# Azure/mmlspark

Measured on NVIDIA H100. Metric: boosting_iters_per_sec, higher is better.
Workload: dtype int64 fixed-point histograms over u8 bins (fp32 gradients, fp64 split gains)

## Files before the change

include/b200gbm_c_api.h:

```cpp
#ifndef B200GBM_C_API_H_
#define B200GBM_C_API_H_

#include <stddef.h>
#include <stdint.h>

#ifdef __cplusplus
extern "C" {
#endif

typedef void* DatasetHandle;
typedef void* BoosterHandle;

#define C_API_DTYPE_FLOAT32 (0)
#define C_API_DTYPE_FLOAT64 (1)
#define C_API_DTYPE_INT32 (2)
#define C_API_DTYPE_INT64 (3)

#define C_API_PREDICT_NORMAL (0)
#define C_API_PREDICT_RAW_SCORE (1)
#define C_API_PREDICT_LEAF_INDEX (2)
#define C_API_PREDICT_CONTRIB (3)

const char* LGBM_GetLastError(void);

// ... 51 lines not shown
                          int64_t buffer_len, int64_t* out_len, char* out_str);

int LGBM_BoosterPredictForMatSingle(BoosterHandle handle, const void* data, int data_type, int ncol, int is_row_major,
                                    int predict_type, int start_iteration, int num_iteration, const char* parameter,
                                    int64_t* out_len, double* out_result);
int LGBM_BoosterPredictForCSRSingle(BoosterHandle handle, const void* indptr, int indptr_type, const int32_t* indices,
                                    const void* data, int data_type, int64_t nindptr, int64_t nelem, int64_t num_col,
                                    int predict_type, int start_iteration, int num_iteration, const char* parameter,
                                    int64_t* out_len, double* out_result);
int LGBM_BoosterPredictForMat(BoosterHandle handle, const void* data, int data_type, int32_t nrow, int32_t ncol,
                              int is_row_major, int predict_type, int start_iteration, int num_iteration,
                              const char* parameter, int64_t* out_len, double* out_result);
int LGBM_BoosterCalcNumPredict(BoosterHandle handle, int num_row, int predict_type, int start_iteration,
                               int num_iteration, int64_t* out_len);

typedef void* ChunkedArrayHandle;
int B200GBM_ChunkedArrayCreate(int data_type, int64_t chunk_size, ChunkedArrayHandle* out);
int B200GBM_ChunkedArrayAdd(ChunkedArrayHandle h, double value);
int B200GBM_ChunkedArrayAddMany(ChunkedArrayHandle h, const void* values, int64_t n);
int64_t B200GBM_ChunkedArrayGetAddCount(ChunkedArrayHandle h);
int64_t B200GBM_ChunkedArrayGetChunksCount(ChunkedArrayHandle h);
int64_t B200GBM_ChunkedArrayGetLastChunkAddCount(ChunkedArrayHandle h);
double B200GBM_ChunkedArrayGetItem(ChunkedArrayHandle h, int64_t chunk, int64_t index, double on_fail);
int B200GBM_ChunkedArrayCoalesceTo(ChunkedArrayHandle h, void* out);
int B200GBM_ChunkedArrayRelease(ChunkedArrayHandle h);
int B200GBM_ChunkedArrayFree(ChunkedArrayHandle h);

int B200GBM_SetDevice(int ordinal);
int B200GBM_GetDevice(int* ordinal);
int B200GBM_DeviceAlloc(size_t bytes, void** out);
int B200GBM_DeviceFree(void* ptr);
int B200GBM_HostAllocPinned(size_t bytes, void** out);
int B200GBM_HostFreePinned(void* ptr);
int B200GBM_Memcpy(void* dst, const void* src, size_t bytes);
int B200GBM_SampleIndices(int num_total_row, int sample_cnt, int seed, int* out, int* out_len);
int B200GBM_SyntheticFill(void* dev_x_f32, void* dev_label_f32, int64_t row_start, int32_t nrow, int32_t ncol,
                          uint64_t seed, int kind);
int B200GBM_SyntheticRows(const int* rows, int32_t nrows, int32_t ncol, uint64_t seed, int kind, double* host_out,
                          float* host_label_out);
int B200GBM_DatasetGetBins(DatasetHandle handle, uint8_t* out_row_major);
int B200GBM_DatasetGetBins16(DatasetHandle handle, uint16_t* out_row_major);
int B200GBM_DatasetGetBinToCat(DatasetHandle handle, int feature, int* out, int* out_len);
int B200GBM_DatasetGetBinsRows(DatasetHandle handle, const int32_t* rows, int32_t nrows, uint16_t* out);
int B200GBM_DatasetGetBundles(DatasetHandle handle, int* out_num_columns, int* out_column_of);
int B200GBM_DatasetGetFeatureRange(DatasetHandle handle, int feature, double* out2);
int B200GBM_DatasetGetFeatureInfo(DatasetHandle handle, int feature, int* out5);
int B200GBM_DatasetGetUpperBounds(DatasetHandle handle, int feature, double* out, int* out_len);
int B200GBM_DatasetGetIngestMs(DatasetHandle handle, double* out_ms);
int B200GBM_DatasetHistogram(DatasetHandle handle, const float* grad, const float* hess, const int32_t* idx,
                             int32_t cnt, double* out);
int B200GBM_BoosterGetGradients(BoosterHandle handle, float* grad, float* hess);
int B200GBM_BoosterSetProfile(BoosterHandle handle, int profile_hist);
int B200GBM_BoosterGetTiming(BoosterHandle handle, double* out6, int reset);
int B200GBM_BoosterGetScores(BoosterHandle handle, int data_idx, double* out);
int B200GBM_BoosterPredictForMatDevice(BoosterHandle handle, const void* data, int data_type, int64_t nrow, int32_t ncol, int predict_type,
                                       int start_iteration, int num_iteration, int64_t* out_len, double* out_result, double* elapsed_ms);
int B200GBM_BoosterPredictForCSRDevice(BoosterHandle handle, const void* indptr, int indptr_type, const int32_t* indices, const void* data,
                                       int data_type, int64_t nindptr, int64_t nelem, int64_t num_col, int predict_type, int start_iteration,
                                       int num_iteration, int64_t* out_len, double* out_result, double* elapsed_ms);
int B200GBM_BoosterGetInfo(BoosterHandle handle, int* out4);
int B200GBM_BoosterGetMemoryInfo(BoosterHandle handle, int64_t* out2);
int B200GBM_BoosterGetColumnCacheInfo(BoosterHandle handle, int64_t* out4);
int B200GBM_BoosterGetCommInfo(BoosterHandle handle, int64_t* out3);

#ifdef __cplusplus
}
#endif
#endif
```

mmlspark_b200/capi.py:

```python
import ctypes as C
import os

import numpy as np

_HERE = os.path.dirname(os.path.abspath(__file__))
LIB_PATH = os.path.join(_HERE, "lib", "libb200gbm.so")
_LIB = None

DTYPE_FLOAT32, DTYPE_FLOAT64, DTYPE_INT32, DTYPE_INT64 = 0, 1, 2, 3
PREDICT_NORMAL, PREDICT_RAW_SCORE, PREDICT_LEAF_INDEX, PREDICT_CONTRIB = 0, 1, 2, 3


class LightGBMError(Exception):
    pass


def load():
    global _LIB
    if _LIB is None:
        if not os.path.exists(LIB_PATH):
            raise LightGBMError(
                "libb200gbm.so is missing (%s). Run `python __graft_entry__.py` to build the CUDA extension; "
                "this package has no CPU fallback." % LIB_PATH)
        L = C.CDLL(LIB_PATH, mode=C.RTLD_GLOBAL)
# ... 393 lines not shown
        X = np.ascontiguousarray(X, dtype=np.float64)
        nrow, ncol = X.shape
        n = C.c_int64(0)
        check(load().LGBM_BoosterCalcNumPredict(self.handle, C.c_int(nrow), C.c_int(predict_type), C.c_int(start_iteration), C.c_int(num_iteration), C.byref(n)))
        out = np.zeros(max(n.value, 1), dtype=np.float64)
        check(load().LGBM_BoosterPredictForMat(self.handle, _ptr(X), C.c_int(DTYPE_FLOAT64), C.c_int32(nrow), C.c_int32(ncol), C.c_int(1), C.c_int(predict_type),
                                               C.c_int(start_iteration), C.c_int(num_iteration), b"", C.byref(n), _ptr(out)))
        return out[:n.value].reshape(nrow, -1)

    def predict_device(self, X, predict_type=PREDICT_NORMAL, start_iteration=0, num_iteration=-1, return_ms=False):
        X = np.ascontiguousarray(X)
        if X.dtype not in (np.float32, np.float64):
            X = X.astype(np.float64)
        nrow, ncol = X.shape
        n = C.c_int64(0)
        check(load().LGBM_BoosterCalcNumPredict(self.handle, C.c_int(nrow), C.c_int(predict_type), C.c_int(start_iteration), C.c_int(num_iteration), C.byref(n)))
        out = np.zeros(max(n.value, 1), dtype=np.float64)
        ms = C.c_double(0)
        check(load().B200GBM_BoosterPredictForMatDevice(self.handle, _ptr(X), C.c_int(_np_dtype_code(X)), C.c_int64(nrow), C.c_int32(ncol), C.c_int(predict_type),
                                                        C.c_int(start_iteration), C.c_int(num_iteration), C.byref(n), _ptr(out), C.byref(ms)))
        res = out[:n.value].reshape(nrow, -1)
        return (res, ms.value) if return_ms else res

    def predict_csr_device(self, indptr, indices=None, data=None, num_col=None, predict_type=PREDICT_NORMAL, start_iteration=0, num_iteration=-1,
                           return_ms=False):
        if not isinstance(indptr, np.ndarray) and hasattr(indptr, "tocsr"):
            m = indptr.tocsr()
            indptr, indices, data, num_col = m.indptr, m.indices, m.data, m.shape[1]
        indptr = np.ascontiguousarray(indptr)
        if indptr.dtype not in (np.int32, np.int64):
            indptr = indptr.astype(np.int64)
        indices = np.ascontiguousarray(indices, dtype=np.int32)
        data = np.ascontiguousarray(data, dtype=np.float64)
        nrow = len(indptr) - 1
        n = C.c_int64(0)
        check(load().LGBM_BoosterCalcNumPredict(self.handle, C.c_int(max(nrow, 0)), C.c_int(predict_type), C.c_int(start_iteration), C.c_int(num_iteration), C.byref(n)))
        out = np.zeros(max(n.value, 1), dtype=np.float64)
        ms = C.c_double(0)
        check(load().B200GBM_BoosterPredictForCSRDevice(self.handle, _ptr(indptr), C.c_int(DTYPE_INT32 if indptr.dtype == np.int32 else DTYPE_INT64),
                                                        _ptr(indices), _ptr(data), C.c_int(DTYPE_FLOAT64), C.c_int64(len(indptr)), C.c_int64(len(data)),
                                                        C.c_int64(num_col), C.c_int(predict_type), C.c_int(start_iteration), C.c_int(num_iteration),
                                                        C.byref(n), _ptr(out), C.byref(ms)))
        res = out[:n.value].reshape(nrow, n.value // max(nrow, 1))
        return (res, ms.value) if return_ms else res

    def set_profile(self, on=True):
        check(load().B200GBM_BoosterSetProfile(self.handle, C.c_int(1 if on else 0)))

    def get_timing(self, reset=False):
        out = np.zeros(6, dtype=np.float64)
        check(load().B200GBM_BoosterGetTiming(self.handle, _ptr(out), C.c_int(1 if reset else 0)))
        return dict(hist_ms=out[0], total_ms=out[1], hist_rows=int(out[2]), hist_launches=int(out[3]), launches=int(out[4]), iterations=int(out[5]))

    def get_info(self):
        out = np.zeros(4, dtype=np.int32)
        check(load().B200GBM_BoosterGetInfo(self.handle, _ptr(out)))
        return dict(num_machines=int(out[0]), rank=int(out[1]), reduce_mode=int(out[2]), constant_hessian=bool(out[3]))

    def get_memory_info(self):
        out = np.zeros(2, dtype=np.int64)
        check(load().B200GBM_BoosterGetMemoryInfo(self.handle, _ptr(out)))
        return dict(partition_column_copy_bytes=int(out[0]), device_free_bytes=int(out[1]))

    def get_column_cache_info(self):
        out = np.zeros(4, dtype=np.int64)
        check(load().B200GBM_BoosterGetColumnCacheInfo(self.handle, _ptr(out)))
        return dict(slots=int(out[0]), slots_used=int(out[1]), builds=int(out[2]), evictions=int(out[3]))

    def get_comm_info(self):
        out = np.zeros(3, dtype=np.int64)
        check(load().B200GBM_BoosterGetCommInfo(self.handle, _ptr(out)))
        return dict(hist_bytes=int(out[0]), record_bytes=int(out[1]), splits=int(out[2]))

    def get_scores(self, data_idx=0):
        n = C.c_int64(0)
        check(load().LGBM_BoosterGetNumPredict(self.handle, C.c_int(data_idx), C.byref(n)))
        out = np.zeros(n.value, dtype=np.float64)
        check(load().B200GBM_BoosterGetScores(self.handle, C.c_int(data_idx), _ptr(out)))
        return out

    def get_gradients(self):
        n = C.c_int64(0)
        check(load().LGBM_BoosterGetNumPredict(self.handle, C.c_int(0), C.byref(n)))
        g = np.zeros(n.value, dtype=np.float32)
        h = np.zeros(n.value, dtype=np.float32)
        check(load().B200GBM_BoosterGetGradients(self.handle, _ptr(g), _ptr(h)))
        return g, h

    def free(self):
        if self.handle:
            check(load().LGBM_BoosterFree(self.handle))
            self.handle = None


class ChunkedArray:

    def __init__(self, dtype_code, chunk_size):
        self.h = C.c_void_p()
        self.dtype_code = dtype_code
        check(load().B200GBM_ChunkedArrayCreate(C.c_int(dtype_code), C.c_int64(chunk_size), C.byref(self.h)))

    def add(self, v): check(load().B200GBM_ChunkedArrayAdd(self.h, C.c_double(v)))

    def add_many(self, arr):
        dt = {0: np.float32, 1: np.float64, 2: np.int32}[self.dtype_code]
        a = np.ascontiguousarray(arr, dtype=dt)
# ... 19 lines not shown
```

mmlspark_b200/csrc/c_api.cu:

```cuda
#include "../../include/b200gbm_c_api.h"

#include <cstring>
#include <mutex>
#include <string>
#include <vector>

#include "engine.cu"

using namespace b200gbm;

static thread_local std::string t_last_error = "Everything is fine";

static int Fail(const char* what) {
  t_last_error = what;
  return -1;
}
#define API_BEGIN() try {
#define API_END()                                                        \
  }                                                                      \
  catch (const std::exception& ex) { return Fail(ex.what()); }           \
  catch (const std::string& ex) { return Fail(ex.c_str()); }             \
  catch (...) { return Fail("unknown exception"); }                      \
  return 0;

// ... 523 lines not shown
int B200GBM_DatasetGetBundles(DatasetHandle handle, int* out_num_columns, int* out_column_of) {
  API_BEGIN();
  DS(handle)->GetBundles(out_num_columns, out_column_of);
  API_END();
}
int B200GBM_DatasetGetFeatureRange(DatasetHandle handle, int feature, double* out2) {
  API_BEGIN();
  const FeatureBins& fb = DS(handle)->mappers.at(feature);
  out2[0] = fb.min_val; out2[1] = fb.max_val;
  API_END();
}
int B200GBM_DatasetGetFeatureInfo(DatasetHandle handle, int feature, int* out5) {
  API_BEGIN();
  const FeatureBins& fb = DS(handle)->mappers.at(feature);
  out5[0] = fb.num_bin; out5[1] = fb.missing_type; out5[2] = static_cast<int>(fb.default_bin); out5[3] = static_cast<int>(fb.most_freq_bin);
  out5[4] = fb.trivial ? 1 : 0;
  API_END();
}
int B200GBM_DatasetGetUpperBounds(DatasetHandle handle, int feature, double* out, int* out_len) {
  API_BEGIN();
  const FeatureBins& fb = DS(handle)->mappers.at(feature);
  for (size_t i = 0; i < fb.upper.size(); ++i) out[i] = fb.upper[i];
  *out_len = static_cast<int>(fb.upper.size());
  API_END();
}
int B200GBM_DatasetGetIngestMs(DatasetHandle handle, double* out_ms) {
  API_BEGIN();
  *out_ms = DS(handle)->ingest_ms;
  API_END();
}
int B200GBM_DatasetHistogram(DatasetHandle handle, const float* grad, const float* hess, const int32_t* idx, int32_t cnt, double* out) {
  API_BEGIN();
  DS(handle)->Histogram(grad, hess, idx, cnt, out);
  API_END();
}
int B200GBM_BoosterGetGradients(BoosterHandle handle, float* grad, float* hess) {
  API_BEGIN();
  BS(handle)->GetGradients(grad, hess);
  API_END();
}
int B200GBM_BoosterSetProfile(BoosterHandle handle, int profile_hist) {
  API_BEGIN();
  BS(handle)->SetProfile(profile_hist != 0);
  API_END();
}
int B200GBM_BoosterGetTiming(BoosterHandle handle, double* out6, int reset) {
  API_BEGIN();
  Booster* b = BS(handle);
  out6[0] = b->timing.hist_ms; out6[1] = b->timing.total_ms; out6[2] = static_cast<double>(b->timing.hist_rows);
  out6[3] = static_cast<double>(b->timing.hist_launches); out6[4] = static_cast<double>(b->timing.launches); out6[5] = b->iter;
  if (reset) b->timing = Booster::Timing();
  API_END();
}
int B200GBM_BoosterPredictForMatDevice(BoosterHandle handle, const void* data, int data_type, int64_t nrow, int32_t ncol, int predict_type,
                                       int start_iteration, int num_iteration, int64_t* out_len, double* out_result, double* elapsed_ms) {
  API_BEGIN();
  Booster* b = BS(handle);
  *out_len = b->PredictBatch(data, data_type, nrow, ncol, predict_type, start_iteration, num_iteration, out_result);
  if (elapsed_ms) *elapsed_ms = b->last_predict_ms;
  API_END();
}
int B200GBM_BoosterPredictForCSRDevice(BoosterHandle handle, const void* indptr, int indptr_type, const int32_t* indices, const void* data,
                                       int data_type, int64_t nindptr, int64_t nelem, int64_t num_col, int predict_type, int start_iteration,
                                       int num_iteration, int64_t* out_len, double* out_result, double* elapsed_ms) {
  API_BEGIN();
  (void)num_col;
  Booster* b = BS(handle);
  *out_len = b->PredictBatchCSR(indptr, indptr_type, indices, data, data_type, nindptr, nelem, predict_type, start_iteration, num_iteration, out_result);
  if (elapsed_ms) *elapsed_ms = b->last_predict_ms;
  API_END();
}
int B200GBM_BoosterGetInfo(BoosterHandle handle, int* out4) {
  API_BEGIN();
  BS(handle)->GetInfo(out4);
  API_END();
}
int B200GBM_BoosterGetMemoryInfo(BoosterHandle handle, int64_t* out2) {
  API_BEGIN();
  BS(handle)->GetMemoryInfo(out2);
  API_END();
}
int B200GBM_BoosterGetColumnCacheInfo(BoosterHandle handle, int64_t* out4) {
  API_BEGIN();
  BS(handle)->GetColumnCacheInfo(out4);
  API_END();
}
int B200GBM_BoosterGetCommInfo(BoosterHandle handle, int64_t* out3) {
  API_BEGIN();
  BS(handle)->GetCommInfo(out3);
  API_END();
}
int B200GBM_BoosterGetScores(BoosterHandle handle, int data_idx, double* out) {
  API_BEGIN();
  BS(handle)->GetRawScores(data_idx, out);
  API_END();
}
}
```

mmlspark_b200/csrc/engine.h:

```cpp
#pragma once
#include <cuda_runtime.h>
#include <nccl.h>

#include <cstdint>
#include <memory>
#include <stdexcept>
#include <map>
#include <mutex>
#include <string>
#include <vector>

#include "bin_mapper.h"
#include "bundle.h"
#include "config.h"
#include "kernels.cuh"
#include "model.h"

namespace b200gbm {

#define B200_CUDA(x)                                                                                      \
  do {                                                                                                    \
    cudaError_t e__ = (x);                                                                                \
    if (e__ != cudaSuccess)                                                                               \
      throw std::runtime_error(std::string("CUDA error: ") + cudaGetErrorString(e__) + " at " + __FILE__ + ":" + std::to_string(__LINE__)); \
// ... 108 lines not shown
  static std::unique_ptr<Dataset> NewShell(int nrow, int ncol, const char* params);
  template <typename Sample> void SetMappers(const Dataset* reference, bool may_bundle, Sample sample);
  template <typename Count> void DissolveConflictingBundles(Count count);
  void UploadBundleMembers();
  std::vector<int> SampleRows() const;
  void AllocBins();
  template <typename T> void UnpackTiles(T* out) const;
  struct MatPart { const void* data; long long nrow; bool on_device; };
  void BinBlock(const std::vector<MatPart>& parts, int data_type, int is_row_major, long long start_row);
  template <typename Fn> void ForEachDeviceBlock(const std::vector<MatPart>& parts, int data_type, int is_row_major, Fn fn);
  DevBuf<unsigned char> ingest_buf_[2];
  cudaStream_t ingest_copy_stream_ = nullptr;
  cudaEvent_t ingest_copied_[2] = {nullptr, nullptr}, ingest_binned_[2] = {nullptr, nullptr};
  long long ingest_rows_done_ = 0;
  void ReleaseIngestStaging();
  void UploadMeta();
  mutable DevBuf<int> block_bound_;
  mutable std::mutex block_bound_mu_;
};

struct ValidSet {
  const Dataset* ds = nullptr;
  DevBuf<double> score;
};
class Objective;
class TreeLearner;
class Metrics;

class Booster {
 public:
  Booster(const Dataset* train, const char* params);
  explicit Booster(const std::string& model_text);
  ~Booster();

  bool UpdateOneIter();
  bool UpdateOneIterCustom(const float* grad, const float* hess);
  void ResetParameter(const char* params);
  void AddValidData(const Dataset* valid);
  void MergeFrom(const Booster* other);
  std::vector<std::string> EvalNames() const;
  std::vector<double> GetEval(int data_idx);
  void GetPredict(int data_idx, int64_t* out_len, double* out);
  int64_t NumPredict(int data_idx) const;
  void GetRawScores(int data_idx, double* out);
  void GetGradients(float* grad, float* hess);
  int64_t PredictBatch(const void* data, int data_type, int64_t nrow, int ncol, int predict_type, int start_iteration, int num_iteration, double* out);
  int64_t PredictBatchCSR(const void* indptr, int indptr_type, const int32_t* indices, const void* data, int data_type, int64_t nindptr,
                          int64_t nelem, int predict_type, int start_iteration, int num_iteration, double* out);
  double last_predict_ms = 0.0;
  void GetInfo(int* out4) const { out4[0] = parallel_ ? Net().world : 1; out4[1] = parallel_ ? Net().rank : 0; out4[2] = same_device_ ? 3 : 0; out4[3] = const_hessian_ ? 1 : 0; }
  std::string SaveModelToString(int start_iteration, int num_iteration, int importance_type) const;
  std::string DumpModelJson(int start_iteration, int num_iteration) const;

  struct Timing { double hist_ms = 0, total_ms = 0; long long hist_rows = 0; long long hist_launches = 0, launches = 0; };
  Timing timing;
  void SetProfile(bool profile_hist);
  void GetMemoryInfo(int64_t* out2);
  void GetColumnCacheInfo(int64_t* out4) const;
  void GetCommInfo(int64_t* out3) const;

  Config cfg;
  HostModel model;
  const Dataset* train = nullptr;
  int K = 1;
  int iter = 0;
  int num_init_iteration = 0;

 private:
  void InitTraining();
  bool TrainTrees(const float* custom_g, const float* custom_h);
  void TrainOneTree(int class_id, HostTree* out);
  double BoostFromAverage(int class_id);

  std::unique_ptr<Objective> obj_;
  std::unique_ptr<TreeLearner> learner_;
  std::unique_ptr<Metrics> metrics_;
  int device_ = 0;
  cudaStream_t stream_ = nullptr;
  bool parallel_ = false;
  bool voting_ = false;
  bool same_device_ = false;
  bool const_hessian_ = false;
  bool has_init_score_ = false;
  double shrinkage_ = 0.1;
  bool is_rf_ = false, is_goss_ = false, bagging_ = false, balanced_bagging_ = false, use_bag_ = false, need_re_bagging_ = false;
  int bag_count_ = 0, bag_blocks_ = 0;
  DevBuf<unsigned> bag_lcg_;
  DevBuf<LcgJump> bag_jump_;
  DevBuf<uint8_t> in_bag_;
  DevBuf<int> bag_block_cnt_, bag_idx_, bag_total_;
  std::vector<double> rf_init_scores_;
  void Bagging(int it);
  void ComputeGradientsAt(const double* score);
  bool is_dart_ = false, dart_dropped_this_iter_ = false;
  LcgRandom drop_rand_{4};
  std::vector<int> drop_index_;
  std::vector<double> tree_weight_;
  double sum_weight_ = 0.0;
  std::vector<std::unique_ptr<DevBuf<unsigned char>>> tree_store_;
  void DroppingTrees();
  void DartNormalize();
  void AddStoredTree(int iter_index, int class_id, bool to_train, bool to_valid);
  DevBuf<double> score_;
  DevBuf<float> grad_, hess_;
  struct SlotBufs { int t0 = 0, t1 = 0, U = 0; DevBuf<int> slot_of_feature, feature_of_slot, split_slot; };
  struct ForestBufs {
    DevBuf<int> tree_offset, leaf_offset, num_leaves, split_feature, decision_type, left_child, right_child, cat_begin, cat_len; DevBuf<double> threshold, leaf_value, node_count, leaf_count, expected; DevBuf<unsigned> cat_words; size_t trees = 0; int max_depth = 0;
// ... 18 lines not shown
```

mmlspark_b200/csrc/hist_kernel.cuh:

```cuda
#pragma once
#include <cstdint>
#include <cuda_runtime.h>
#include <cub/block/block_scan.cuh>

namespace b200gbm {

constexpr int kTileFeat = 32;
constexpr int kBins = 256;
constexpr int kLoBits = 18;
constexpr int kFlushRows = 1 << (32 - kLoBits);
#ifndef B200GBM_K4_EXPERIMENT
#define B200GBM_K4_EXPERIMENT 0
#endif
constexpr int kPlaneWords = kBins * kTileFeat;

struct HistWork {
  int begin;
  int count;
  int use_idx;
  int buf;
};

__global__ void __launch_bounds__(256)
k_gather_q(const HistWork* __restrict__ work, const int* __restrict__ idx0, const int* __restrict__ idx1, const int4* __restrict__ qgh,
// ... 35 lines not shown
  __syncthreads();
  const int ncol = min(kTileFeat, num_columns - tile * kTileFeat);
  unsigned m = 0u;
  for (int e = tid; e < kBins * kTileFeat; e += blockDim.x)
    if ((e & (kTileFeat - 1)) < ncol) m = max(m, cnt[e]);
  m = __reduce_max_sync(0xffffffffu, m);
  if ((tid & 31) == 0) wmax[tid >> 5] = m;
  __syncthreads();
  if (tid == 0) {
    for (int i = 1; i < static_cast<int>(blockDim.x >> 5); ++i) m = max(m, wmax[i]);
    prefix[static_cast<size_t>(tile) * (gridDim.x + 1) + blockIdx.x] = static_cast<int>(m);
  }
}

__global__ void __launch_bounds__(1024) k_block_bound_prefix(int blocks, int* __restrict__ prefix) {
  using Scan = cub::BlockScan<int, 1024>;
  __shared__ typename Scan::TempStorage tmp;
  int* p = prefix + static_cast<size_t>(blockIdx.x) * (blocks + 1);
  int carry = 0;
  for (int b0 = 0; b0 < blocks; b0 += 1024) {
    const int b = b0 + threadIdx.x;
    const int v = b < blocks ? p[b] : 0;
    int ex, total;
    Scan(tmp).ExclusiveSum(v, ex, total);
    if (b < blocks) p[b] = carry + ex;
    carry += total;
    __syncthreads();
  }
  if (threadIdx.x == 0) p[blocks] = carry;
}

inline void launch_block_bound(const uint8_t* bins, size_t rows_stride, int num_data, int num_tiles, int num_columns, int* prefix,
                               cudaStream_t stream) {
  const int blocks = bound_blocks(num_data);
  if (blocks > 0) k_block_maxcnt<<<dim3(blocks, num_tiles), 256, 0, stream>>>(bins, rows_stride, num_data, num_columns, prefix);
  k_block_bound_prefix<<<num_tiles, 1024, 0, stream>>>(blocks, prefix);
}


__device__ __forceinline__ void cp_async16(void* smem, const void* gmem, bool valid) {
  unsigned s = static_cast<unsigned>(__cvta_generic_to_shared(smem));
  int sz = valid ? 16 : 0;
  asm volatile("cp.async.cg.shared.global [%0], [%1], 16, %2;\n" ::"r"(s), "l"(gmem), "r"(sz));
}
template <int N>
__device__ __forceinline__ void cp_async_wait() {
  asm volatile("cp.async.wait_group %0;\n" ::"n"(N));
}

constexpr int kWsConsumerWarps = 16;
constexpr int kWsProducerWarps = 2;
constexpr int kWsThreads = (kWsConsumerWarps + kWsProducerWarps) * 32;
constexpr int kWsStageRows = 512;
constexpr int kWsStages = 3;
constexpr int kFlushSlabBins = 32;
constexpr int kFlushRowBytes = kFlushSlabBins * 16;
constexpr int kFlushStageBytes = kTileFeat * kFlushRowBytes;
constexpr int kWsSmemBytes = 4 * kPlaneWords * 4 + kWsStages * (kWsStageRows * 32 + kWsStageRows * 16) + kFlushStageBytes + 64;
static_assert(kWsSmemBytes <= 227 * 1024, "K4 shared memory exceeds the 227 KB per block of sm_90");
static_assert(kFlushSlabBins * kTileFeat == 2 * kWsConsumerWarps * 32, "a flush slab is two (g,h) pairs per consumer thread");

__device__ __forceinline__ unsigned smem_u32(const void* p) { return static_cast<unsigned>(__cvta_generic_to_shared(p)); }
__device__ __forceinline__ void mbar_init(unsigned long long* bar, unsigned count) {
  asm volatile("mbarrier.init.shared::cta.b64 [%0], %1;\n" ::"r"(smem_u32(bar)), "r"(count));
}
__device__ __forceinline__ void mbar_arrive(unsigned long long* bar) {
  asm volatile("mbarrier.arrive.shared::cta.b64 _, [%0];\n" ::"r"(smem_u32(bar)) : "memory");
}
__device__ __forceinline__ void mbar_arrive_expect_tx(unsigned long long* bar, unsigned bytes) {
  asm volatile("mbarrier.arrive.expect_tx.shared::cta.b64 _, [%0], %1;\n" ::"r"(smem_u32(bar)), "r"(bytes) : "memory");
}
__device__ __forceinline__ void mbar_expect_tx(unsigned long long* bar, unsigned bytes) {
  asm volatile("mbarrier.expect_tx.relaxed.cta.shared::cta.b64 [%0], %1;\n" ::"r"(smem_u32(bar)), "r"(bytes) : "memory");
}
__device__ __forceinline__ void mbar_wait(unsigned long long* bar, unsigned parity) {
  asm volatile(
      "{\n"
      ".reg .pred p;\n"
      "WAIT_LOOP:\n"
      "mbarrier.try_wait.parity.shared::cta.b64 p, [%0], %1;\n"
      "@p bra DONE;\n"
      "bra WAIT_LOOP;\n"
      "DONE:\n"
      "}\n" ::"r"(smem_u32(bar)), "r"(parity) : "memory");
}
__device__ __forceinline__ void tma_bulk_g2s(void* smem_dst, const void* gmem_src, unsigned bytes, unsigned long long* bar) {
  asm volatile("cp.async.bulk.shared::cluster.global.mbarrier::complete_tx::bytes [%0], [%1], %2, [%3];\n" ::"r"(smem_u32(smem_dst)),
               "l"(gmem_src), "r"(bytes), "r"(smem_u32(bar))
               : "memory");
}
__device__ __forceinline__ void cp_async_mbar_arrive_noinc(unsigned long long* bar) {
  asm volatile("cp.async.mbarrier.arrive.noinc.shared::cta.b64 [%0];\n" ::"r"(smem_u32(bar)) : "memory");
}
__device__ __forceinline__ void bulk_reduce_add_u64(unsigned long long* gmem_dst, const void* smem_src, unsigned bytes) {
  asm volatile("cp.reduce.async.bulk.global.shared::cta.bulk_group.add.u64 [%0], [%1], %2;\n" ::"l"(gmem_dst), "r"(smem_u32(smem_src)),
               "r"(bytes)
               : "memory");
}
__device__ __forceinline__ void bulk_commit() { asm volatile("cp.async.bulk.commit_group;\n" ::: "memory"); }
__device__ __forceinline__ void bulk_wait_read_all() { asm volatile("cp.async.bulk.wait_group.read 0;\n" ::: "memory"); }
__device__ __forceinline__ void bulk_wait_all() { asm volatile("cp.async.bulk.wait_group 0;\n" ::: "memory"); }
__device__ __forceinline__ void fence_proxy_async_smem() { asm volatile("fence.proxy.async.shared::cta;\n" ::: "memory"); }

template <int NATOM>
__global__ void __launch_bounds__(kWsThreads, 1)
k4_hist_build_ws(const uint8_t* __restrict__ bins, size_t rows_stride, int num_tiles, const int4* __restrict__ qgh,
                 const int4* __restrict__ qord, const int* __restrict__ idx0, const int* __restrict__ idx1,
                 const HistWork* __restrict__ work, unsigned long long* __restrict__ hist, RowBlockBound bound) {
  extern __shared__ __align__(128) unsigned char smem_raw[];
  unsigned* plane = reinterpret_cast<unsigned*>(smem_raw);
  unsigned char* stage_bins = smem_raw + 4 * kPlaneWords * 4;
  int4* stage_q = reinterpret_cast<int4*>(stage_bins + kWsStages * kWsStageRows * 32);
  unsigned char* flush_stage = reinterpret_cast<unsigned char*>(stage_q) + kWsStages * kWsStageRows * 16;
  unsigned long long* full_bar = reinterpret_cast<unsigned long long*>(flush_stage + kFlushStageBytes);
  unsigned long long* empty_bar = full_bar + kWsStages;

  const HistWork w = *work;
  const int n = w.count;
  if (n <= 0) return;
  const int tid = threadIdx.x, lane = tid & 31, warp = tid >> 5;
  const int* __restrict__ idx = w.buf ? idx1 : idx0;

  long long cells_rows = static_cast<long long>(n) * num_tiles;
  int rpi = static_cast<int>((cells_rows + 4LL * gridDim.x - 1) / (4LL * gridDim.x));
  rpi = (rpi + kWsStageRows - 1) / kWsStageRows * kWsStageRows;
  rpi = max(rpi, kWsStageRows);
  rpi = min(rpi, kFlushRows);
  const int chunks = (n + rpi - 1) / rpi;
  const long long items = static_cast<long long>(chunks) * num_tiles;
  const int i0 = static_cast<int>(items * blockIdx.x / gridDim.x);
  const int i1 = static_cast<int>(items * (blockIdx.x + 1) / gridDim.x);
  if (i0 >= i1) return;

  if (tid == 0) {
    for (int i = 0; i < kWsStages; ++i) { mbar_init(&full_bar[i], kWsProducerWarps * 32); mbar_init(&empty_bar[i], kWsConsumerWarps); }
    asm volatile("fence.mbarrier_init.release.cluster;\n" ::: "memory");
  }
  for (int e = tid; e < 4 * kPlaneWords; e += kWsThreads) plane[e] = 0u;
  __syncthreads();

  unsigned gs = 0;
  if (warp >= kWsConsumerWarps) {
    const int ptid = tid - kWsConsumerWarps * 32;
    constexpr int kPT = kWsProducerWarps * 32;
    constexpr int kPerLane = kWsStageRows / kPT;
    for (int item = i0; item < i1; ++item) {
      const int tile = item / chunks, chunk = item - tile * chunks;
      const int row0 = chunk * rpi;
      const int nrows = min(rpi, n - row0);
      const int nst = (nrows + kWsStageRows - 1) / kWsStageRows;
      const uint8_t* tbins = bins + static_cast<size_t>(tile) * rows_stride * 32;
      for (int s = 0; s < nst; ++s, ++gs) {
        const int slot = gs % kWsStages;
        mbar_wait(&empty_bar[slot], ((gs / kWsStages) & 1u) ^ 1u);
        const int p0 = row0 + s * kWsStageRows;
        const int rows = min(kWsStageRows, row0 + nrows - p0);
        unsigned char* db = stage_bins + slot * kWsStageRows * 32;
        int4* dq = stage_q + slot * kWsStageRows;
        if (!w.use_idx) {
          if (ptid == 0) {
            mbar_arrive_expect_tx(&full_bar[slot], static_cast<unsigned>(rows) * 48u);
            const size_t r = static_cast<size_t>(w.begin + p0);
            tma_bulk_g2s(db, tbins + r * 32, static_cast<unsigned>(rows) * 32u, &full_bar[slot]);
            tma_bulk_g2s(dq, qgh + r, static_cast<unsigned>(rows) * 16u, &full_bar[slot]);
          } else {
            mbar_arrive(&full_bar[slot]);
          }
        } else {
          const int* ip = idx + w.begin + p0;
          if (ptid == 0) {
            mbar_expect_tx(&full_bar[slot], static_cast<unsigned>(rows) * 16u);
            tma_bulk_g2s(dq, qord + static_cast<size_t>(w.begin + p0), static_cast<unsigned>(rows) * 16u, &full_bar[slot]);
          }
          int rr[2 * kPerLane];
#pragma unroll
          for (int k = 0; k < 2 * kPerLane; ++k) { const int j = (ptid + k * kPT) >> 1; rr[k] = j < rows ? ip[j] : -1; }
#pragma unroll
          for (int k = 0; k < 2 * kPerLane; ++k) {
            const int hh = ptid + k * kPT, j = hh >> 1, half = (hh & 1) * 16;
            if (rr[k] >= 0) cp_async16(db + j * 32 + half, tbins + static_cast<size_t>(rr[k]) * 32 + half, true);
          }
          cp_async_mbar_arrive_noinc(&full_bar[slot]);
        }
      }
// ... 150 lines not shown
```

mmlspark_b200/csrc/kernels.cuh:

```cuda
#pragma once
#include <climits>
#include <cstdint>
#include <cuda_runtime.h>
#include "config.h"
#include "hist_kernel.cuh"

namespace b200gbm {

constexpr double kEpsD = 1e-15;
#define kNegInf (-__longlong_as_double(0x7ff0000000000000LL))

struct FeatMeta {
  int num_bin;
  int missing_type;
  int default_bin;
  int offset;
  int real_index;
  int is_categorical;
  int num_sorted_cats;
  int hist_off;
  int table_off;
};

__host__ __device__ __forceinline__ unsigned d_unbundle(unsigned slot, int base, int mfb, int num_bin) {
// ... 29 lines not shown
  int interaction;
  double path_smooth;
};

__host__ __device__ __forceinline__ unsigned d_lcg_next(unsigned x) { return 214013u * x + 2531011u; }
__device__ __forceinline__ int d_extra_draw(unsigned* x, int range) {
  if (range <= 0) return 0;
  *x = d_lcg_next(*x);
  return static_cast<int>((*x & 0x7fffffffu) % static_cast<unsigned>(range));
}
__global__ void k_extra_seed(unsigned* __restrict__ xrand, const int* __restrict__ pos, int nf, int extra_seed) {
  for (int u = blockIdx.x * blockDim.x + threadIdx.x; u < nf; u += gridDim.x * blockDim.x) xrand[u] = static_cast<unsigned>(extra_seed + pos[u]);
}
__device__ __forceinline__ int d_cat_rand_range(int used_bin, int max_cat_threshold) {
  const int max_num_cat = min(max_cat_threshold, (used_bin + 1) / 2);
  return max(min(max_num_cat, used_bin) - 1, 0);
}

struct SplitCand {
  double gain;
  double left_g, left_h;
  int threshold, left_count, default_left, feature;
  double l2_extra;
  unsigned cat_bits[8];
  int is_cat, cat_list_len;
  unsigned short cat_list[kCatListMax];
};

struct LeafBest {
  double gain;
  double left_g, left_h, right_g, right_h;
  double left_out, right_out;
  int feature, threshold, default_left, left_count, right_count, is_cat;
  unsigned cat_bits[8];
  int cat_list_len, monotone_type;
  unsigned short cat_list[kCatListMax];
  unsigned long long inter_sets;
};

struct LeafState {
  int begin, count, buf, depth;
  int global_count, identity, hist_slot, parent_node;
  double sum_g, sum_h;
  LeafBest best;
  long long qtot[2], qpar[2];
  double mono_min, mono_max;
  double output;
  unsigned long long inter_mask;
};

struct ConstraintArgs { const signed char* type; double penalty; const unsigned long long* sets_of; };
struct NodeSampleArgs { uint8_t* mask; int* work; const int* order; const uint8_t* tree_used; int k; };

struct TreeCtrl {
  int num_leaves, left_leaf, right_leaf, smaller, larger, go, finished, split_leaf;
  int split_feature, split_threshold, split_default_left, split_missing_type, split_num_bin, new_leaf, pending, pad;
  int part_begin, part_count, part_buf, part_identity, part_left_total, smaller_rows, round, split_is_cat;
  unsigned split_cat_bits[8];
  HistWork hist_work;
  unsigned absmax_bits[2];
  int exp_g, exp_h;
  double inv_g, inv_h;
  long long root_q[4];
  long long trace_rows;
  unsigned scan_ticket;
  int q_side;
  unsigned part_barrier;
  unsigned part_ticket;
  unsigned part_next[2];
  int split_wide;
  int split_cat_list_len;
  unsigned short split_cat_list[kCatListMax];
  unsigned col_state, col_next;
};

struct TreeDev {
  int* left_child; int* right_child; int* split_feature_inner; int* threshold_bin; int* decision_type;
  float* split_gain; double* leaf_value; double* leaf_weight; int* leaf_count; double* internal_value;
  double* internal_weight; int* internal_count; int* leaf_parent; int* leaf_depth; int* num_leaves;
  unsigned* cat_bits;
  unsigned short* cat_list;
  int* cat_list_len;
};

__device__ __forceinline__ double d_sign(double x) { return (x > 0.0) - (x < 0.0); }
__device__ __forceinline__ double d_threshold_l1(double s, double l1) {
  double r = fmax(0.0, fabs(s) - l1);
  return d_sign(s) * r;
}
__device__ __forceinline__ double d_calc_output(double g, double h, const SplitParams& p) {
  double ret = (p.l1 > 0) ? -d_threshold_l1(g, p.l1) / (h + p.l2) : -g / (h + p.l2);
  if (p.max_delta_step > 0 && fabs(ret) > p.max_delta_step) ret = d_sign(ret) * p.max_delta_step;
  return ret;
}
__device__ __noinline__ double d_leaf_gain(double g, double h, const SplitParams& p) {
  if (!(p.max_delta_step > 0)) {
    if (p.l1 > 0) { double sg = d_threshold_l1(g, p.l1); return (sg * sg) / (h + p.l2); }
    return (g * g) / (h + p.l2);
  }
  double out = d_calc_output(g, h, p);
  double sg = (p.l1 > 0) ? d_threshold_l1(g, p.l1) : g;
  return -(2.0 * sg * out + (h + p.l2) * out * out);
}
__device__ __noinline__ double d_smooth_output(double g, double h, int n, double parent_output, const SplitParams& p) {
  double ret = d_calc_output(g, h, p);
  if (p.path_smooth > kPathSmoothEps) {
    const double w = n / p.path_smooth;
    ret = ret * w / (w + 1) + parent_output / (w + 1);
  }
  return ret;
}
__device__ __noinline__ double d_smooth_leaf_gain(double g, double h, int n, double parent_output, const SplitParams& p) {
  if (!(p.path_smooth > kPathSmoothEps)) return d_leaf_gain(g, h, p);
  const double out = d_smooth_output(g, h, n, parent_output, p);
  const double sg = (p.l1 > 0) ? d_threshold_l1(g, p.l1) : g;
  return -(2.0 * sg * out + (h + p.l2) * out * out);
}
__device__ __forceinline__ double d_mono_output(double g, double h, int n, double parent_output, const SplitParams& p, double lo, double hi) {
  double ret = d_smooth_output(g, h, n, parent_output, p);
  if (ret < lo) ret = lo;
  else if (ret > hi) ret = hi;
  return ret;
}
__device__ __noinline__ double d_mono_split_gain(double lg, double lh, double rg, double rh, int lc, int rc, double parent_output, const SplitParams& p,
                                                 double lo, double hi, int mono) {
  const double lo_out = d_mono_output(lg, lh, lc, parent_output, p, lo, hi), ro_out = d_mono_output(rg, rh, rc, parent_output, p, lo, hi);
// ... 550 lines not shown
      tree.leaf_value[leaf] = isnan(b.left_out) ? 0.0 : b.left_out;
      tree.leaf_weight[leaf] = b.left_h; tree.leaf_count[leaf] = b.left_count;
      tree.leaf_value[nl] = isnan(b.right_out) ? 0.0 : b.right_out;
      tree.leaf_weight[nl] = b.right_h; tree.leaf_count[nl] = b.right_count;
      tree.leaf_depth[nl] = tree.leaf_depth[leaf] + 1; tree.leaf_depth[leaf] += 1;
      const FeatMeta fm = meta[b.feature];
      if (b.is_cat) {
        tree.decision_type[node] = 1 | (fm.missing_type << 2);
        tree.threshold_bin[node] = 0;
      } else {
        tree.decision_type[node] = (b.default_left ? 2 : 0) | (fm.missing_type << 2);
        tree.threshold_bin[node] = b.threshold;
      }
      for (int wd = 0; wd < 8; ++wd) tree.cat_bits[node * 8 + wd] = b.is_cat ? b.cat_bits[wd] : 0u;
      tree.cat_list_len[node] = b.is_cat ? b.cat_list_len : 0;
      if (b.is_cat) for (int k = 0; k < b.cat_list_len && k < kCatListMax; ++k) tree.cat_list[node * kCatListMax + k] = b.cat_list[k];
      ctrl->num_leaves += 1; *tree.num_leaves = ctrl->num_leaves;
      const int dst_buf = L.identity ? 0 : (L.buf ^ 1);
      R.begin = L.begin + true_left; R.count = true_right; R.buf = dst_buf; R.identity = 0; R.depth = L.depth + 1;
      L.count = true_left; L.buf = dst_buf; L.identity = 0; L.depth += 1;
      L.global_count = b.left_count; R.global_count = b.right_count;
      L.sum_g = b.left_g; L.sum_h = b.left_h; R.sum_g = b.right_g; R.sum_h = b.right_h;
      d_constrain_children(L, R, b.monotone_type, b.is_cat, b.left_out, b.right_out, p.interaction, L.best.inter_sets);
      R.hist_slot = nl;
      L.best.gain = kNegInf; L.best.feature = -1; R.best.gain = kNegInf; R.best.feature = -1;
      ctrl->left_leaf = leaf; ctrl->right_leaf = nl;
    }
    ctrl->go = 0; ctrl->smaller = -1; ctrl->larger = -1; ctrl->split_leaf = -1;
    ctrl->hist_work.count = 0; ctrl->part_count = 0;
    if (!ctrl->finished && !last && ctrl->num_leaves < p.num_leaves) {
      const int ll = ctrl->left_leaf, rl = ctrl->right_leaf;
      bool go = true;
      if (p.max_depth > 0 && tree.leaf_depth[ll] >= p.max_depth) go = false;
      const int nl_cnt = leaves[ll].global_count, nr_cnt = rl >= 0 ? leaves[rl].global_count : 0;
      if (go && nr_cnt < p.min_data_in_leaf * 2 && nl_cnt < p.min_data_in_leaf * 2) go = false;
      if (!go) {
        leaves[ll].best.gain = kNegInf;
        if (rl >= 0) leaves[rl].best.gain = kNegInf;
      } else {
        int smaller = ll, larger = -1;
        if (rl >= 0) {
          if (nl_cnt < nr_cnt) { smaller = ll; larger = rl; } else { smaller = rl; larger = ll; }
          if (larger == rl) { int t = leaves[ll].hist_slot; leaves[ll].hist_slot = leaves[rl].hist_slot; leaves[rl].hist_slot = t; }
          s_copy[0] = ll; s_copy[1] = rl;
        }
        ctrl->smaller = smaller; ctrl->larger = larger; ctrl->go = 1;
        const LeafState& S = leaves[smaller];
        ctrl->hist_work.begin = S.begin; ctrl->hist_work.count = S.count; ctrl->hist_work.use_idx = S.identity ? 0 : 1;
        ctrl->hist_work.buf = S.buf;
        ctrl->smaller_rows = S.count;
        ctrl->trace_rows += S.count;
      }
    }
    ctrl->round += 1;
  }
  __syncthreads();
  if (s_copy[0] >= 0)
    for (int u = threadIdx.x; u < p.nf_pad; u += blockDim.x) flags[static_cast<size_t>(s_copy[1]) * p.nf_pad + u] = flags[static_cast<size_t>(s_copy[0]) * p.nf_pad + u];
}
__global__ void __launch_bounds__(256)
k_round_ctl(TreeCtrl* ctrl, LeafState* leaves, TreeDev tree, uint8_t* flags, const FeatMeta* __restrict__ meta, SplitParams p,
            int last) {
  __shared__ int s_copy[2];
  d_round_ctl(ctrl, leaves, tree, flags, meta, p, last, s_copy);
}



__device__ __noinline__ bool d_smaller_drew_cat(const long long* __restrict__ hist, int num_bin, const LeafState& S, double inv_h,
                                                const SplitParams& p, int max_cat_threshold) {
  const double cnt_factor = S.global_count / (S.sum_h + 2 * kEpsD);
  int used_bin = 0;
  for (int b0 = 0; b0 < num_bin; b0 += blockDim.x) {
    const int b = b0 + threadIdx.x;
    bool used = false;
    if (b >= 1 && b < num_bin) used = static_cast<int>(static_cast<double>(hist[b * 2 + 1]) * inv_h * cnt_factor + 0.5) >= p.cat_smooth;
    used_bin += __syncthreads_count(used);
  }
  return d_cat_rand_range(used_bin, max_cat_threshold) > 0;
}
__device__ __forceinline__ bool d_smaller_drew(const long long* __restrict__ hist, const FeatMeta& m, const TreeCtrl* ctrl, const LeafState* leaves,
                                               const SplitParams& p, int max_cat_threshold) {
  if (!m.is_categorical) return m.num_bin > 2;
  if (m.num_bin <= p.max_cat_to_onehot) return m.num_bin > 1;
  return d_smaller_drew_cat(hist, m.num_bin, leaves[ctrl->smaller], ctrl->inv_h, p, max_cat_threshold);
}

template <bool kExtra, typename Next, typename Visit>
__device__ __forceinline__ void d_cat_walk(int used_bin, int max_num_cat, int num_data, double sum_h, double cnt_factor, const SplitParams& p,
                                           int rand_i, Next next, Visit visit) {
  int cnt_cur_group = 0, left_count = 0;
  double slg = 0.0, slh = kEpsD;
  for (int i = 0; i < used_bin && i < max_num_cat; ++i) {
    double g, h;
    next(&g, &h);
    const int cnt = static_cast<int>(h * cnt_factor + 0.5);
    slg += g; slh += h; left_count += cnt; cnt_cur_group += cnt;
    if (left_count < p.min_data_in_leaf || slh < p.min_sum_hessian) continue;
    const int right_count = num_data - left_count;
    if (right_count < p.min_data_in_leaf || right_count < p.min_data_per_group) break;
    const double srh = sum_h - slh;
    if (srh < p.min_sum_hessian) break;
    if (cnt_cur_group < p.min_data_per_group) continue;
    cnt_cur_group = 0;
    if (kExtra && i != rand_i) continue;
    visit(i, slg, slh, srh, left_count);
// ... 1823 lines not shown
```

mmlspark_b200/csrc/tree_learner.cu:

```cuda
#include "tree_learner.h"

namespace b200gbm {

static size_t Align16(size_t x) { return (x + 15) & ~static_cast<size_t>(15); }
constexpr int kScanSmem = (768 + 64) * 8;
constexpr int kPartTickets = 8;

static int SampleCount(int total, double fraction) { return std::max(static_cast<int>(total * fraction + 0.5), std::min(2, total)); }

struct ScanKernels {
  decltype(&k_scan<kScanPlain>) scan;
  decltype(&k_scan_wide<false, false>) scan_wide;
};
static const ScanKernels kScanKernels[2][2] = {
    {{k_scan<kScanPlain, false, false>, k_scan_wide<false, false>}, {k_scan<kScanPlain, false, true>, k_scan_wide<false, true>}},
    {{k_scan<kScanPlain, true, false>, k_scan_wide<true, false>}, {k_scan<kScanPlain, true, true>, k_scan_wide<true, true>}}};

template <typename Fn>
static void ForEachTreeField(TreeDev& t, int L, Fn fn) {
  const size_t nodes = L - 1, leaves = L;
  fn(t.left_child, nodes); fn(t.right_child, nodes); fn(t.split_feature_inner, nodes); fn(t.threshold_bin, nodes);
  fn(t.decision_type, nodes); fn(t.split_gain, nodes); fn(t.leaf_value, leaves); fn(t.leaf_weight, leaves); fn(t.leaf_count, leaves);
  fn(t.internal_value, nodes); fn(t.internal_weight, nodes); fn(t.internal_count, nodes); fn(t.leaf_parent, leaves);
  fn(t.leaf_depth, leaves); fn(t.num_leaves, 1); fn(t.cat_bits, 8 * nodes); fn(t.cat_list, kCatListMax * nodes); fn(t.cat_list_len, nodes);
// ... 403 lines not shown
      comm_rec_bytes_ += static_cast<long long>(all_recs_.n * sizeof(VoteRec));
      timing_.launches += 2;
    } else {
      nvtxRangePushA(parallel_ ? "b200gbm:C2 histogram reduce + K5 scan + pick" : "b200gbm:K5 scan + pick");
      if (parallel_) {
        Net().AllReduce(H_.p, slot_elems_, ncclInt64, ncclSum, s);
        comm_hist_bytes_ += static_cast<long long>(slot_elems_ * sizeof(long long));
      }
      mark();
      const ScanKernels& k = kScanKernels[extra_trees_][monotone_ || smooth_];
      if (d.nw > 0) {
        k.scan_wide<<<dim3(d.nw, 2), 256, kWideMaxBins * 8, s>>>(ctrl, leaves_.p, d.meta.p, H_.p, pool_.p, slot_elems_, flags_.p, cands_.p, sp_, xrand_.p,
                                                                 cons);
        timing_.launches += 1;
      }
      const NodeSampleArgs node = bynode_ ? NodeSampleArgs{node_mask_.p, node_work_.p, real_order_.p, feature_used_.p, bynode_k_} : NodeSampleArgs{};
      k.scan<<<sgrid, 256, scan_smem, s>>>(ctrl, leaves_.p, d.meta.p, H_.p, pool_.p, slot_elems_, flags_.p, cands_.p, sp_, d.BundleBase(), VoteBufs{}, xrand_.p,
                                           cons, node);
      nvtxRangePop();
    }
    mark();
    comm_splits_ += 1;
    nvtxRangePushA("b200gbm:K7 partition + controller");
    LaunchPartition(pgrid, split == L - 2 ? 1 : 0);
    nvtxRangePop();
    mark();
    timing_.launches += 3; timing_.hist_launches += 1;
  }
}

void TreeLearner::AddScore(double* score_k, double shrinkage) {
  k_add_score<<<num_sms_ * 8, 256, 0, stream_>>>(ctrl_.p, leaves_.p, tree_dev_, idx0_.p, idx1_.p, score_k, shrinkage);
}

void TreeLearner::ReadTree(HostTree* out) {
  const Dataset& d = train_;
  cudaStream_t s = stream_;
  B200_CUDA(cudaMemcpyAsync(tree_host_, tree_blob_.p, tree_blob_.n, cudaMemcpyDeviceToHost, s));
  B200_CUDA(cudaMemcpyAsync(ctrl_host_, ctrl_.p, sizeof(TreeCtrl), cudaMemcpyDeviceToHost, s));
  B200_CUDA(cudaStreamSynchronize(s));
  if (!split_events_.empty()) {
    static const char* kOps[] = {"gather_q(bagged root)", "K4", "allreduce", "scan+pick", "partition+zeroH+ctl"};
    static const char* kVotingOps[] = {"gather_q(bagged root)", "K4", "local scan+top-k", "allgather", "vote+pack", "allreduce", "global scan+pick",
                                       "partition+zeroH+ctl"};
    const char* const* ops = voting_ ? kVotingOps : kOps;
    const int per = voting_ ? 9 : 6;
    for (size_t b0 = 0; b0 + per <= split_events_.size(); b0 += per)
      for (int o = 0; o < per - 1; ++o) { float ms = 0; cudaEventElapsedTime(&ms, split_events_[b0 + o], split_events_[b0 + o + 1]); split_op_ms_[ops[o]] += ms; }
    split_op_trees_ += 1;
    for (auto e : split_events_) cudaEventDestroy(e);
    split_events_.clear();
  }
  if (!hist_events_.empty()) {
    for (size_t i = 0; i + 1 < hist_events_.size(); i += 2) { float ms = 0; cudaEventElapsedTime(&ms, hist_events_[i], hist_events_[i + 1]); timing_.hist_ms += ms; }
    for (auto e : hist_events_) cudaEventDestroy(e);
    hist_events_.clear();
  }
  timing_.hist_rows += ctrl_host_->trace_rows;
  col_rand_.set_state(ctrl_host_->col_state);
  const TreeDev t = TreeAt(tree_host_);
  const int nl = *t.num_leaves;
  out->Resize(nl);
  if (nl > 1) {
    for (int i = 0; i < nl - 1; ++i) {
      const int sf = t.split_feature_inner[i], tb = t.threshold_bin[i], dt = t.decision_type[i];
      out->left_child[i] = t.left_child[i]; out->right_child[i] = t.right_child[i]; out->split_feature_inner[i] = sf;
      out->split_feature[i] = d.used[sf]; out->threshold_in_bin[i] = static_cast<uint32_t>(tb);
      out->decision_type[i] = static_cast<int8_t>(dt); out->split_gain[i] = t.split_gain[i];
      const FeatureBins& fbm = d.mappers[d.used[sf]];
      if (dt & 1) {
        std::vector<int> cats;
        if (sf >= d.nfn) { for (int k = 0; k < t.cat_list_len[i]; ++k) cats.push_back(fbm.bin_to_cat[t.cat_list[i * kCatListMax + k]]); }
        else for (int b = 0; b < fbm.num_bin; ++b) if ((t.cat_bits[i * 8 + (b >> 5)] >> (b & 31)) & 1u) cats.push_back(fbm.bin_to_cat[b]);
        out->AddCategoricalNode(i, cats);
      } else {
        double thr = fbm.upper[tb];
        if (std::isnan(thr)) thr = 0.0; else if (thr >= 1e300) thr = 1e300; else if (thr <= -1e300) thr = -1e300;
        out->threshold[i] = thr;
      }
      out->internal_value[i] = t.internal_value[i]; out->internal_weight[i] = t.internal_weight[i]; out->internal_count[i] = t.internal_count[i];
    }
    for (int i = 0; i < nl; ++i) { out->leaf_value[i] = t.leaf_value[i]; out->leaf_weight[i] = t.leaf_weight[i]; out->leaf_count[i] = t.leaf_count[i]; out->leaf_depth[i] = t.leaf_depth[i]; }
  } else {
    out->leaf_value[0] = 0.0;
  }
  UpdateColumnCache(*out);
}

}
```

Before: 6.493.

## Assign histogram blocks to per-tile row bands for indexed launches, add launch tracing

When the histogram launch uses a row index and there are at least 16 feature tiles with enough blocks, each block now takes one tile and a contiguous band of row chunks. This replaces the flat split of chunk-by-tile items, aiming for better locality and fewer flush conflicts per tile. It also adds per-round tracing: two 512-entry int arrays in TreeCtrl written each round, plus a host API to read per-launch timings. The tracing grows the control struct copied back to the host after every tree.

```diff
diff --git a/include/b200gbm_c_api.h b/include/b200gbm_c_api.h
--- a/include/b200gbm_c_api.h
+++ b/include/b200gbm_c_api.h
@@ -127,6 +127,8 @@
 int B200GBM_BoosterGetGradients(BoosterHandle handle, float* grad, float* hess);
 int B200GBM_BoosterSetProfile(BoosterHandle handle, int profile_hist);
 int B200GBM_BoosterGetTiming(BoosterHandle handle, double* out6, int reset);
+int B200GBM_BoosterGetHistLaunches(BoosterHandle handle, int64_t capacity, int64_t* out_len, double* out_ms, int32_t* out_rows,
+                                   int32_t* out_use_idx);
 int B200GBM_BoosterGetScores(BoosterHandle handle, int data_idx, double* out);
 int B200GBM_BoosterPredictForMatDevice(BoosterHandle handle, const void* data, int data_type, int64_t nrow, int32_t ncol, int predict_type,
                                        int start_iteration, int num_iteration, int64_t* out_len, double* out_result, double* elapsed_ms);
diff --git a/mmlspark_b200/capi.py b/mmlspark_b200/capi.py
--- a/mmlspark_b200/capi.py
+++ b/mmlspark_b200/capi.py
@@ -469,6 +469,13 @@
         check(load().B200GBM_BoosterGetTiming(self.handle, _ptr(out), C.c_int(1 if reset else 0)))
         return dict(hist_ms=out[0], total_ms=out[1], hist_rows=int(out[2]), hist_launches=int(out[3]), launches=int(out[4]), iterations=int(out[5]))
 
+    def get_hist_launches(self):
+        n = C.c_int64(0)
+        check(load().B200GBM_BoosterGetHistLaunches(self.handle, C.c_int64(0), C.byref(n), None, None, None))
+        ms, rows, use_idx = np.zeros(max(n.value, 1)), np.zeros(max(n.value, 1), dtype=np.int32), np.zeros(max(n.value, 1), dtype=np.int32)
+        check(load().B200GBM_BoosterGetHistLaunches(self.handle, C.c_int64(n.value), C.byref(n), _ptr(ms), _ptr(rows), _ptr(use_idx)))
+        return dict(ms=ms[:n.value], rows=rows[:n.value], use_idx=use_idx[:n.value])
+
     def get_info(self):
         out = np.zeros(4, dtype=np.int32)
         check(load().B200GBM_BoosterGetInfo(self.handle, _ptr(out)))
diff --git a/mmlspark_b200/csrc/c_api.cu b/mmlspark_b200/csrc/c_api.cu
--- a/mmlspark_b200/csrc/c_api.cu
+++ b/mmlspark_b200/csrc/c_api.cu
@@ -599,6 +599,16 @@
   if (reset) b->timing = Booster::Timing();
   API_END();
 }
+int B200GBM_BoosterGetHistLaunches(BoosterHandle handle, int64_t capacity, int64_t* out_len, double* out_ms, int32_t* out_rows,
+                                   int32_t* out_use_idx) {
+  API_BEGIN();
+  const Booster::Timing& t = BS(handle)->timing;
+  *out_len = static_cast<int64_t>(t.launch_ms.size());
+  for (size_t i = 0; i < t.launch_ms.size() && static_cast<int64_t>(i) < capacity; ++i) {
+    out_ms[i] = t.launch_ms[i]; out_rows[i] = t.launch_rows[i]; out_use_idx[i] = t.launch_use_idx[i];
+  }
+  API_END();
+}
 int B200GBM_BoosterPredictForMatDevice(BoosterHandle handle, const void* data, int data_type, int64_t nrow, int32_t ncol, int predict_type,
                                        int start_iteration, int num_iteration, int64_t* out_len, double* out_result, double* elapsed_ms) {
   API_BEGIN();
diff --git a/mmlspark_b200/csrc/engine.h b/mmlspark_b200/csrc/engine.h
--- a/mmlspark_b200/csrc/engine.h
+++ b/mmlspark_b200/csrc/engine.h
@@ -184,7 +184,10 @@
   std::string SaveModelToString(int start_iteration, int num_iteration, int importance_type) const;
   std::string DumpModelJson(int start_iteration, int num_iteration) const;
 
-  struct Timing { double hist_ms = 0, total_ms = 0; long long hist_rows = 0; long long hist_launches = 0, launches = 0; };
+  struct Timing {
+    double hist_ms = 0, total_ms = 0; long long hist_rows = 0; long long hist_launches = 0, launches = 0;
+    std::vector<float> launch_ms; std::vector<int> launch_rows, launch_use_idx;
+  };
   Timing timing;
   void SetProfile(bool profile_hist);
   void GetMemoryInfo(int64_t* out2);
diff --git a/mmlspark_b200/csrc/hist_kernel.cuh b/mmlspark_b200/csrc/hist_kernel.cuh
--- a/mmlspark_b200/csrc/hist_kernel.cuh
+++ b/mmlspark_b200/csrc/hist_kernel.cuh
@@ -111,6 +111,7 @@
 constexpr int kWsProducerWarps = 2;
 constexpr int kWsThreads = (kWsConsumerWarps + kWsProducerWarps) * 32;
 constexpr int kWsStageRows = 512;
+constexpr int kBandMinTiles = 16;
 constexpr int kWsStages = 3;
 constexpr int kFlushSlabBins = 32;
 constexpr int kFlushRowBytes = kFlushSlabBins * 16;
@@ -187,8 +188,14 @@
   rpi = min(rpi, kFlushRows);
   const int chunks = (n + rpi - 1) / rpi;
   const long long items = static_cast<long long>(chunks) * num_tiles;
-  const int i0 = static_cast<int>(items * blockIdx.x / gridDim.x);
-  const int i1 = static_cast<int>(items * (blockIdx.x + 1) / gridDim.x);
+  int i0 = static_cast<int>(items * blockIdx.x / gridDim.x);
+  int i1 = static_cast<int>(items * (blockIdx.x + 1) / gridDim.x);
+  if (w.use_idx && num_tiles >= kBandMinTiles && static_cast<int>(gridDim.x) >= num_tiles) {
+    const int t = blockIdx.x % num_tiles, band = blockIdx.x / num_tiles;
+    const int bands = (static_cast<int>(gridDim.x) - t + num_tiles - 1) / num_tiles;
+    i0 = t * chunks + static_cast<int>(static_cast<long long>(chunks) * band / bands);
+    i1 = t * chunks + static_cast<int>(static_cast<long long>(chunks) * (band + 1) / bands);
+  }
   if (i0 >= i1) return;
 
   if (tid == 0) {
diff --git a/mmlspark_b200/csrc/kernels.cuh b/mmlspark_b200/csrc/kernels.cuh
--- a/mmlspark_b200/csrc/kernels.cuh
+++ b/mmlspark_b200/csrc/kernels.cuh
@@ -105,6 +105,7 @@
 struct ConstraintArgs { const signed char* type; double penalty; const unsigned long long* sets_of; };
 struct NodeSampleArgs { uint8_t* mask; int* work; const int* order; const uint8_t* tree_used; int k; };
 
+constexpr int kTraceRounds = 512;
 struct TreeCtrl {
   int num_leaves, left_leaf, right_leaf, smaller, larger, go, finished, split_leaf;
   int split_feature, split_threshold, split_default_left, split_missing_type, split_num_bin, new_leaf, pending, pad;
@@ -125,6 +126,8 @@
   int split_cat_list_len;
   unsigned short split_cat_list[kCatListMax];
   unsigned col_state, col_next;
+  int trace_count[kTraceRounds];
+  int trace_use_idx[kTraceRounds];
 };
 
 struct TreeDev {
@@ -781,6 +784,7 @@
         ctrl->trace_rows += S.count;
       }
     }
+    if (ctrl->round < kTraceRounds) { ctrl->trace_count[ctrl->round] = ctrl->hist_work.count; ctrl->trace_use_idx[ctrl->round] = ctrl->hist_work.use_idx; }
     ctrl->round += 1;
   }
   __syncthreads();
diff --git a/mmlspark_b200/csrc/tree_learner.cu b/mmlspark_b200/csrc/tree_learner.cu
--- a/mmlspark_b200/csrc/tree_learner.cu
+++ b/mmlspark_b200/csrc/tree_learner.cu
@@ -479,7 +479,15 @@
     split_events_.clear();
   }
   if (!hist_events_.empty()) {
-    for (size_t i = 0; i + 1 < hist_events_.size(); i += 2) { float ms = 0; cudaEventElapsedTime(&ms, hist_events_[i], hist_events_[i + 1]); timing_.hist_ms += ms; }
+    for (size_t i = 0; i + 1 < hist_events_.size(); i += 2) {
+      float ms = 0;
+      cudaEventElapsedTime(&ms, hist_events_[i], hist_events_[i + 1]);
+      timing_.hist_ms += ms;
+      if (i / 2 >= static_cast<size_t>(kTraceRounds)) continue;
+      timing_.launch_ms.push_back(ms);
+      timing_.launch_rows.push_back(ctrl_host_->trace_count[i / 2]);
+      timing_.launch_use_idx.push_back(ctrl_host_->trace_use_idx[i / 2]);
+    }
     for (auto e : hist_events_) cudaEventDestroy(e);
     hist_events_.clear();
   }
```

Measured after the change: 6.563 (median of 6 runs). +1.1%, better.
